# ZhengyiLuo/UHC

Hardware: AMD Instinct MI355X
Metric: env-steps/sec (69-DoF SMPL humanoid, 15 substeps/step) (higher is better)
Workload: dtype f64

## Files before the change

uhc_amd/csrc/uhc_device.h:

```cpp
#pragma once
#include <hip/hip_runtime.h>
#include <stdint.h>

#define UHC_WAVE 64
#define UHC_FAST_MAXEFC 64
#define UHC_FAST_MAXCON 16
#define UHC_FAST_MAXCON_DENSE 24
#define UHC_FAST_MAXTWO 12
#define UHC_GEN_MAXEFC 128
#define UHC_GEN_MAXCON 64
#define UHC_GEN_MAXTWO 20
#define UHC_BIG_MAXEFC 256
#define UHC_BIG_MAXCON 128
#define UHC_BIG_MAXTWO 32
#define UHC_MAXTWO 32
#define UHC_HUGE_MAXEFC 1024
#define UHC_HUGE_MAXCON 192
#define UHC_HUGE_MAXCON_MOST 320
#define UHC_HUGE_MAXTWO 128
#define UHC_DOF_MAXACT 4
#define UHC_CON_STRIDE 24
#define UHC_WHY_CONTACTS (1 << 16)
#define UHC_WHY_ROWS (1 << 17)
#define UHC_WHY_DENSE_SLOTS (1 << 18)
// ... 126 lines not shown
    int last_tier;
    const int* order;
    int tier_want;
    int sticky_mask;
    int* list;
    int* list_count;
    int* list_cursor;
    const int* prod_fin;
    int prod_total;
    int n_wait;
    int* spares;
    int* started;
    int* fin;
    int* q_next;
    int* q_next_count;
    const int* guard_tab;
    int* guard_hits;
    int* cnt4;
    int grid;
    int marks[8];
    int t4_rows;
    int truncate;
    int ball_limits;
    int dbg;
    int nvp;
    int adjdeg;
    DevCtrl c;
    DevState s;
    int n_env;
    int chunk;
    int* ticket;
    int* chunk_done;
    int* chunk_rec;
};
#define UHC_CHUNK_ALL 0x7fff
#define UHC_CHUNK_ABANDON (1 << 30)
#define UHC_CHUNK_TAKEN (1 << 29)
#define UHC_CHUNK_CLOSING (1 << 28)
#define UHC_CHUNK_REC 16
```

uhc_amd/csrc/uhc_mpr.h:

```cpp
#pragma once

#define UHC_CCD_EPS 2.220446049250313e-16
#define UHC_MPR_TOLERANCE 1e-6
#define UHC_MPR_MAXIT 50
#define UHC_MPR_MAXSUP 256

struct V3 { double x, y, z; };
__device__ __forceinline__ V3 v3(double x, double y, double z) { V3 r = {x, y, z}; return r; }
__device__ __forceinline__ V3 operator-(const V3& a, const V3& b) { return v3(a.x - b.x, a.y - b.y, a.z - b.z); }
__device__ __forceinline__ V3 operator+(const V3& a, const V3& b) { return v3(a.x + b.x, a.y + b.y, a.z + b.z); }
__device__ __forceinline__ V3 operator*(const V3& a, double s) { return v3(a.x * s, a.y * s, a.z * s); }
__device__ __forceinline__ V3 neg(const V3& a) { return v3(-a.x, -a.y, -a.z); }
__device__ __forceinline__ double vdot(const V3& a, const V3& b) { return a.x * b.x + a.y * b.y + a.z * b.z; }
__device__ __forceinline__ V3 vcross(const V3& a, const V3& b) { return v3(a.y * b.z - a.z * b.y, a.z * b.x - a.x * b.z, a.x * b.y - a.y * b.x); }
__device__ __forceinline__ V3 vnorm(const V3& a) { const double n = sqrt(vdot(a, a)); return v3(a.x / n, a.y / n, a.z / n); }
__device__ __forceinline__ V3 vsel(bool c, const V3& a, const V3& b) { return v3(c ? a.x : b.x, c ? a.y : b.y, c ? a.z : b.z); }
__device__ __forceinline__ bool ccd_zero(double x) { return fabs(x) < UHC_CCD_EPS; }
__device__ __forceinline__ bool ccd_eq(double a, double b) {
    const double ab = fabs(a - b);
    if (ab < UHC_CCD_EPS) return true;
    a = fabs(a); b = fabs(b);
    return b > a ? ab < UHC_CCD_EPS * b : ab < UHC_CCD_EPS * a;
}

// ... 362 lines not shown
                if (cont) dir = vnorm(vcross(p1.v - p0.v, p2.v - p0.v));
                else { p3 = v4; to_refine = true; }
            }
        } else if (st == MPR_REFINE) {
            dt = vdot(v4.v, dir);
            if (!(ccd_zero(dt) || dt > 0) || portal_reach_tolerance(p1, p2, p3, v4, dir)) st = MPR_DONE;
            else { expand_portal(p0, p1, p2, p3, v4); to_refine = true; }
        } else if (st == MPR_PEN) {
            if (portal_reach_tolerance(p1, p2, p3, v4, dir) || it > UHC_MPR_MAXIT) {
                V3 pd;
                M.depth = sqrt(point_tri_dist2(p1.v, p2.v, p3.v, pd));
                if (ccd_zero(pd.x) && ccd_zero(pd.y) && ccd_zero(pd.z)) pd = dir;
                M.dir = vnorm(pd);
                M.pos = find_pos(p0, p1, p2, p3);
                M.hit = true;
                st = MPR_DONE;
            } else {
                expand_portal(p0, p1, p2, p3, v4);
                it++;
                dir = portal_dir(p1, p2, p3);
            }
        }
        if (to_refine) {
            dir = portal_dir(p1, p2, p3);
            dt = vdot(dir, p1.v);
            if (ccd_zero(dt) || dt > 0) to_pen = true;
            else st = MPR_REFINE;
        }
        if (to_pen) { dir = portal_dir(p1, p2, p3); it = 0; st = MPR_PEN; }
    }
}

#if defined(UHC_NW2)
enum { MCMD_EXIT = 0, MCMD_ROUND = 1, MCMD_ROWS = 2 };
struct MprMB { int* hdr; double* io[6]; double* hm1; double* hm2; int* st4; int* st2; };
template <int TIER>
__device__ __forceinline__ MprMB mpr_mb(const KernelArgs& A, double* S) {
    const DevLds& L = lds_of<TIER>(A);
    MprMB m;
    m.hdr = (int*)(S + L.rowR);
    m.io[0] = S + L.rowR + 4;
    m.io[1] = S + L.rowAref; m.io[2] = S + L.rowAref + UHC_WAVE;
    m.io[3] = S + L.rowB; m.io[4] = S + L.rowB + UHC_WAVE;
    m.io[5] = S + L.rowF; m.hm1 = S + L.rowF + UHC_WAVE;
    m.st4 = (int*)(S + L.rowDa); m.st2 = (int*)(S + L.rowW); m.hm2 = S + L.rowW + UHC_WAVE;
    return m;
}
__device__ __forceinline__ SupArgs mpr_mb_args(const MprMB& MB, const double* xmat, const double* xpos, int p) {
    SupArgs a;
    const int b1 = __builtin_amdgcn_readfirstlane(MB.st4[4 * p]), b2 = __builtin_amdgcn_readfirstlane(MB.st4[4 * p + 1]);
    a.R1 = xmat + 9 * b1; a.P1 = xpos + 3 * b1; a.R2 = xmat + 9 * b2; a.P2 = xpos + 3 * b2;
    a.voff1 = __builtin_amdgcn_readfirstlane(MB.st4[4 * p + 2]); a.vn1 = __builtin_amdgcn_readfirstlane(MB.st4[4 * p + 3]);
    a.voff2 = __builtin_amdgcn_readfirstlane(MB.st2[2 * p]); a.vn2 = __builtin_amdgcn_readfirstlane(MB.st2[2 * p + 1]);
    a.hm1 = MB.hm1[p]; a.hm2 = MB.hm2[p];
    a.d = v3(MB.io[0][p], MB.io[1][p], MB.io[2][p]);
    return a;
}
__device__ __forceinline__ void mpr_mb_put(const MprMB& MB, int p, const V3& a, const V3& b) {
    if (LANE == 0) {
        MB.io[0][p] = a.x - b.x; MB.io[1][p] = a.y - b.y; MB.io[2][p] = a.z - b.z; MB.io[3][p] = a.x + b.x; MB.io[4][p] = a.y + b.y; MB.io[5][p] = a.z + b.z;
    }
}
__device__ __forceinline__ void mpr_serve_round(const double* __restrict__ VB, const double* __restrict__ xmat, const double* __restrict__ xpos, const MprMB& MB, unsigned long long live, int wid, int nw) {
    const int n = __builtin_popcountll(live), h = (n + nw - 1) / nw;
    int take = min(h, n - wid * h);
    for (int k = 0; k < wid * h && live; k++) live &= live - 1;
    while (live && take > 0) {
// ... 88 lines not shown
                }
                if (cont) dir = vnorm(vcross(p1.v - p0.v, p2.v - p0.v));
                else { p3 = v4; to_refine = true; }
            }
        } else if (st == MPR_REFINE) {
            dt = vdot(v4.v, dir);
            if (!(ccd_zero(dt) || dt > 0) || portal_reach_tolerance(p1, p2, p3, v4, dir)) st = MPR_DONE;
            else { expand_portal(p0, p1, p2, p3, v4); to_refine = true; }
        } else if (st == MPR_PEN) {
            if (portal_reach_tolerance(p1, p2, p3, v4, dir) || it > UHC_MPR_MAXIT) {
                V3 pd;
                M.depth = sqrt(point_tri_dist2(p1.v, p2.v, p3.v, pd));
                if (ccd_zero(pd.x) && ccd_zero(pd.y) && ccd_zero(pd.z)) pd = dir;
                M.dir = vnorm(pd);
                M.pos = find_pos(p0, p1, p2, p3);
                M.hit = true;
                st = MPR_DONE;
            } else {
                expand_portal(p0, p1, p2, p3, v4);
                it++;
                dir = portal_dir(p1, p2, p3);
            }
        }
        if (to_refine) {
            dir = portal_dir(p1, p2, p3);
            dt = vdot(dir, p1.v);
            if (ccd_zero(dt) || dt > 0) to_pen = true;
            else st = MPR_REFINE;
        }
        if (to_pen) { dir = portal_dir(p1, p2, p3); it = 0; st = MPR_PEN; }
    }
}
template <int TIER>
__device__ __forceinline__ void mpr_helper(const KernelArgs& A, double* S) {
    const DevLds& L = lds_of<TIER>(A);
    const MprMB MB = mpr_mb<TIER>(A, S);
    const int* mbi = MB.hdr;
    const int wid = __builtin_amdgcn_readfirstlane((int)(threadIdx.x >> 6));
    const LaneConst HLC = lane_const<true>(A.t);
    for (;;) {
        __syncthreads();
        const int cmd = __builtin_amdgcn_readfirstlane(mbi[0]);
        if (cmd == MCMD_EXIT) return;
        if (cmd == MCMD_ROWS) {
            const int nefc = __builtin_amdgcn_readfirstlane(mbi[1]), ntwo = __builtin_amdgcn_readfirstlane(mbi[2]);
            const unsigned long long mbp = ((unsigned long long)(unsigned)__builtin_amdgcn_readfirstlane(mbi[5]) << 32) | (unsigned)__builtin_amdgcn_readfirstlane(mbi[4]);
            __syncthreads();
            if (ntwo > 0) k_dense_groups<TIER>(A, S, HLC, S + L.dense, ntwo, 1, 2);
            __syncthreads();
            if (UHC_WAVE + LANE < nefc) k_row_one<TIER>(A, (const double*)mbp, S, UHC_WAVE + LANE, S + L.Y);
            __syncthreads();
            continue;
        }
        const unsigned long long live = ((unsigned long long)(unsigned)__builtin_amdgcn_readfirstlane(mbi[2]) << 32) | (unsigned)__builtin_amdgcn_readfirstlane(mbi[1]);
        const int vst = __builtin_amdgcn_readfirstlane(mbi[3]);
        if (vst >= 0) mpr_serve_round(S + vst, S + L.xmat, S + L.xpos, MB, live, wid, UHC_NWG);
        else {
            const unsigned long long vb = ((unsigned long long)(unsigned)__builtin_amdgcn_readfirstlane(mbi[5]) << 32) | (unsigned)__builtin_amdgcn_readfirstlane(mbi[4]);
            mpr_serve_round((const double*)vb, S + L.xmat, S + L.xpos, MB, live, wid, UHC_NWG);
        }
        __syncthreads();
    }
}
template <int TIER>
__device__ __forceinline__ void mpr_release_helpers(const KernelArgs& A, double* S) {
    int* mbi = mpr_mb<TIER>(A, S).hdr;
    if (LANE == 0) mbi[0] = MCMD_EXIT;
    __syncthreads();
}
#endif
```

uhc_amd/csrc/uhc_physics_impl.h:

```cpp
#pragma once
#include <type_traits>
#include "../../include/uhc_amd.h"
#include "uhc_device.h"

extern __shared__ __attribute__((aligned(16))) double smem[];

#if defined(UHC_NW4)
#define UHC_NWG 4
#elif defined(UHC_NW2)
#define UHC_NWG 2
#else
#define UHC_NWG 1
#endif
#if UHC_NWG > 1
#define LANE ((int)(threadIdx.x & 63u))
#else
#define LANE ((int)threadIdx.x)
#endif
#define UHC_NPROF 40
#ifdef UHC_STAGE_PROF
#define PROF_DECL long long pt_[UHC_NPROF] = {}; long long pt_last_ = __builtin_readcyclecounter();
#define PROF_ARGS , long long* pt_, long long& pt_last_
#define PROF_PASS , pt_, pt_last_
#define PROF(i) { const long long now_ = __builtin_readcyclecounter(); pt_[i] += now_ - pt_last_; pt_last_ = now_; }
// ... 35 lines not shown
    int lo = __builtin_amdgcn_readlane(__double2loint(v), src);
    int hi = __builtin_amdgcn_readlane(__double2hiint(v), src);
    return __hiloint2double(hi, lo);
}
template <int CTRL>
__device__ __forceinline__ double dpp_f64(double v) {
    const int lo = __builtin_amdgcn_update_dpp(0, __double2loint(v), CTRL, 0xf, 0xf, true);
    const int hi = __builtin_amdgcn_update_dpp(0, __double2hiint(v), CTRL, 0xf, 0xf, true);
    return __hiloint2double(hi, lo);
}
#define DPP_QUAD_1032 0xB1
#define DPP_QUAD_2301 0x4E
#define DPP_ROW_HALF_MIRROR 0x141
#define DPP_ROW_MIRROR 0x140
__device__ __forceinline__ double wave_sum(double v) {
    v += dpp_f64<DPP_QUAD_1032>(v);
    v += dpp_f64<DPP_QUAD_2301>(v);
    v += dpp_f64<DPP_ROW_HALF_MIRROR>(v);
    v += dpp_f64<DPP_ROW_MIRROR>(v);
    return (bcast(v, 0) + bcast(v, 16)) + (bcast(v, 32) + bcast(v, 48));
}
__device__ __forceinline__ double wave_min(double v) {
    v = fmin(v, dpp_f64<DPP_QUAD_1032>(v));
    v = fmin(v, dpp_f64<DPP_QUAD_2301>(v));
    v = fmin(v, dpp_f64<DPP_ROW_HALF_MIRROR>(v));
    v = fmin(v, dpp_f64<DPP_ROW_MIRROR>(v));
    return fmin(fmin(bcast(v, 0), bcast(v, 16)), fmin(bcast(v, 32), bcast(v, 48)));
}
__device__ __forceinline__ int wave_or(int v) { return __builtin_amdgcn_ballot_w64(v != 0) != 0; }
template <int TIER> __device__ __forceinline__ void k_row_one(const KernelArgs& A, const double* mb, double* S, const int r, double* Yb);
struct LaneConst { int d0, d1, n0, n1, m0, m1, pk0, pk1, r0, r1; bool v0, v1; };
template <int TIER> __device__ __forceinline__ void k_dense_groups(const KernelArgs& A, double* S, const LaneConst& LC, double* Db, const int ntwo, const int first, const int stride);
template <bool DENSE> __device__ __forceinline__ LaneConst lane_const(const DevTopo& T);
#include "uhc_mpr.h"

__device__ __forceinline__ void cross3(double* r, const double* a, const double* b) {
    double r0 = a[1] * b[2] - a[2] * b[1], r1 = a[2] * b[0] - a[0] * b[2], r2 = a[0] * b[1] - a[1] * b[0];
    r[0] = r0; r[1] = r1; r[2] = r2;
}
__device__ __forceinline__ double dot3(const double* a, const double* b) { return a[0] * b[0] + a[1] * b[1] + a[2] * b[2]; }
__device__ __forceinline__ void quat_mul(double* r, const double* a, const double* b) {
    double t0 = a[0] * b[0] - a[1] * b[1] - a[2] * b[2] - a[3] * b[3];
    double t1 = a[0] * b[1] + a[1] * b[0] + a[2] * b[3] - a[3] * b[2];
    double t2 = a[0] * b[2] - a[1] * b[3] + a[2] * b[0] + a[3] * b[1];
    double t3 = a[0] * b[3] + a[1] * b[2] - a[2] * b[1] + a[3] * b[0];
    r[0] = t0; r[1] = t1; r[2] = t2; r[3] = t3;
}
__device__ __forceinline__ void quat_normalize(double* q) {
    double n = sqrt(q[0] * q[0] + q[1] * q[1] + q[2] * q[2] + q[3] * q[3]);
    if (n < UHC_MINVAL) { q[0] = 1; q[1] = q[2] = q[3] = 0; return; }
    double inv = 1.0 / n;
    q[0] *= inv; q[1] *= inv; q[2] *= inv; q[3] *= inv;
}
__device__ __forceinline__ void quat_to_mat(double* m, const double* q) {
    double w = q[0], x = q[1], y = q[2], z = q[3];
    m[0] = w * w + x * x - y * y - z * z; m[1] = 2 * (x * y - w * z); m[2] = 2 * (x * z + w * y);
    m[3] = 2 * (x * y + w * z); m[4] = w * w - x * x + y * y - z * z; m[5] = 2 * (y * z - w * x);
    m[6] = 2 * (x * z - w * y); m[7] = 2 * (y * z + w * x); m[8] = w * w - x * x - y * y + z * z;
}
__device__ __forceinline__ void mat_vec(double* r, const double* m, const double* v) {
    double t0 = m[0] * v[0] + m[1] * v[1] + m[2] * v[2];
    double t1 = m[3] * v[0] + m[4] * v[1] + m[5] * v[2];
    double t2 = m[6] * v[0] + m[7] * v[1] + m[8] * v[2];
    r[0] = t0; r[1] = t1; r[2] = t2;
}
__device__ __forceinline__ void axis_angle_quat(double* q, const double* axis, double angle) {
// ... 1524 lines not shown
        unsigned long long Fb = Fm;
        asm volatile("" : "+s"(Fb));
        static_for<0, NC>([&](auto kc) __attribute__((always_inline)) {
            constexpr int k = NC - 1 - decltype(kc)::value;
            if ((Fb >> k) & 1ull) {
                const double xk = bcast(acc * mypinv, k);
                f = ln == k ? xk : f;
                acc = fma(-W[k], xk, acc);
            }
        });
        PROF(27)
        double y = b;
        unsigned long long Fy = Fm;
        asm volatile("" : "+s"(Fy));
        static_for<0, NC>([&](auto sc) __attribute__((always_inline)) {
            constexpr int s = decltype(sc)::value;
            if ((Fy >> s) & 1ull) y = fma(__hiloint2double(agpr_get(Ahi[s]), agpr_get(Alo[s])), bcast(f, s), y);
        });
        PROF(28)
        const bool bad = valid && (inF ? f < 0.0 : y < 0.0);
        const unsigned long long Bm = __builtin_amdgcn_ballot_w64(bad);
        if (Bm == 0ull) { f_out = f; return it; }
        const int nbad = __builtin_popcountll(Bm);
        bool all = true;
        if (nbad < best) { best = nbad; grace = 3; }
        else if (grace > 0) grace--;
        else all = false;
        const int last = 63 - __builtin_clzll(Bm);
        if (bad && (all || LANE == last)) inF = !inF;
    }
    return -1;
}

template <int LT, bool DENSE>
__device__ __forceinline__ int k_pgs_fast(const KernelArgs& A, const double* mb, double* S, int nefc, FastRow& row, const double (&Y)[UHC_YM], const LaneConst& LC,
                                          const int* SL, int nslot PROF_ARGS) {
    const DevTopo& T = A.t;
    const DevLds& L = lds_of<LT>(A);
    const bool valid = LANE < nefc;
    int ntwo = 0;
    if constexpr (DENSE) {
        for (int k = 0; k < nslot; k++) ntwo += (unsigned)SL[k] < (unsigned)nefc;
        ntwo = __builtin_amdgcn_readfirstlane(ntwo);
    }
    if (DENSE && ntwo > 0) {
        unsigned int cdq[UHC_YM];
        const unsigned int* chain = T.chain + (size_t)(row.last >= 0 ? row.last : 0) * UHC_YM;
        static_for<0, UHC_YM>([&](auto qc) __attribute__((always_inline)) { constexpr int q = decltype(qc)::value; cdq[q] = chain[q] & 0xffffu; });
        for (int k = 0; k < nslot; k++) {
            if ((unsigned)__builtin_amdgcn_readfirstlane(SL[k]) >= (unsigned)nefc) continue;
            const double* Dk = S + L.dense + k * A.nvp;
            double acc = 0.0;
            static_for<0, UHC_YM>([&](auto qc) __attribute__((always_inline)) {
                constexpr int q = decltype(qc)::value;
                acc = fma(Y[q], Dk[cdq[q]], acc);
            });
            S[L.dcol + k * UHC_WAVE + LANE] = valid ? acc : 0.0;
        }
        wsync();
        for (int k = 0; k < nslot; k++) {
            const int lk = __builtin_amdgcn_readfirstlane(SL[k]);
            if ((unsigned)lk >= (unsigned)nefc) continue;
            const double* Dk = S + L.dense + k * A.nvp;
            const double dk0 = LC.v0 ? Dk[LANE] : 0.0, dk1 = LC.v1 ? Dk[LANE + UHC_WAVE] : 0.0;
            for (int m = 0; m <= k; m++) {
                const int lm = __builtin_amdgcn_readfirstlane(SL[m]);
                if ((unsigned)lm >= (unsigned)nefc) continue;
                const double* Dm = S + L.dense + m * A.nvp;
                const double v = wave_sum(dk0 * (LC.v0 ? Dm[LANE] : 0.0) + dk1 * (LC.v1 ? Dm[LANE + UHC_WAVE] : 0.0));
                if (LANE == 0) { S[L.dcol + k * UHC_WAVE + lm] = v; S[L.dcol + m * UHC_WAVE + lk] = v; }
            }
        }
        wsync();
    }
    unsigned int ncp[UHC_WAVE / 4];
    {
        int nraw[UHC_WAVE];
        static_for<0, UHC_WAVE>([&](auto sc) __attribute__((always_inline)) {
            constexpr int s = decltype(sc)::value;
            nraw[s] = 0;
            if (s < nefc) {
                const int ls = __builtin_amdgcn_readlane(row.last, s);
                nraw[s] = (valid && row.last >= 0 && ls >= 0) ? (int)A.t.dof_ncommon[row.last * T.nv + ls] : 0;
            }
        });
        static_for<0, UHC_WAVE / 4>([&](auto jc) __attribute__((always_inline)) {
            constexpr int j = decltype(jc)::value;
            ncp[j] = (unsigned)nraw[4 * j] | ((unsigned)nraw[4 * j + 1] << 8) | ((unsigned)nraw[4 * j + 2] << 16) | ((unsigned)nraw[4 * j + 3] << 24);
        });
    }
    double Ym[UHC_YM];
    int Alo[UHC_WAVE], Ahi[UHC_WAVE];
    double diag = 1.0;
    int prev = -1;
    static_for<0, UHC_YM>([&](auto qc) __attribute__((always_inline)) { Ym[decltype(qc)::value] = 0.0; });
    auto build_A = [&](auto dense_c) __attribute__((always_inline)) {
    constexpr bool DCOL = decltype(dense_c)::value;
    static_for<0, UHC_WAVE>([&](auto sc) __attribute__((always_inline)) {
        constexpr int s = decltype(sc)::value;
        double acc = 0.0;
        if (s < nefc) {
            const int ls = __builtin_amdgcn_readlane(row.last, s);
            const int lens = __builtin_amdgcn_readlane(row.len, s);
            const int two_s = DCOL ? __builtin_amdgcn_readlane(row.two, s) : -1;
            if (DCOL && two_s >= 0) acc = S[L.dcol + two_s * UHC_WAVE + LANE];
            else {
            const double* Ys = S + L.Y + __builtin_amdgcn_readlane(row.yoff, s);
            if (ls != prev) {
                prev = ls;
                const int nc = (ncp[s / 4] >> (8 * (s % 4))) & 0xff;
                static_for<0, UHC_YM>([&](auto qc) __attribute__((always_inline)) {
                    constexpr int q = decltype(qc)::value;
                    Ym[q] = q < nc ? Y[q] : 0.0;
                });
            }
            static_for<0, UHC_YM / 8>([&](auto cc) __attribute__((always_inline)) {
                constexpr int c = decltype(cc)::value;
                if (8 * c < lens) {
                    double y8[8];
                    static_for<0, 8>([&](auto qc) __attribute__((always_inline)) { constexpr int j = decltype(qc)::value; y8[j] = Ys[8 * c + j]; });
                    static_for<0, 8>([&](auto qc) __attribute__((always_inline)) {
                        constexpr int j = decltype(qc)::value;
                        acc = fma(Ym[8 * c + j], y8[j], acc);
// ... 92 lines not shown
    const double f = row.f;
    PROF(11)
    for (int i = LANE; i < T.nv; i += UHC_WAVE) S[L.z + i] = 0.0;
    wsync();
    if (valid && row.last >= 0) {
        const unsigned int* chain = T.chain + (size_t)row.last * UHC_YM;
        const double* Yr = S + L.Y + row.yoff;
        static_for<0, UHC_YM>([&](auto qc) __attribute__((always_inline)) {
            constexpr int q = decltype(qc)::value;
            if (q < row.len) __hip_atomic_fetch_add(S + L.z + (chain[q] & 0xffffu), f * Yr[q], __ATOMIC_RELAXED, __HIP_MEMORY_SCOPE_WORKGROUP);
        });
    }
    wsync();
    if (DENSE && ntwo > 0) {
        for (int k = 0; k < nslot; k++) {
            const int ln = __builtin_amdgcn_readfirstlane(SL[k]);
            if ((unsigned)ln >= (unsigned)nefc) continue;
            const double fk = bcast(f, ln);
            const double* Dk = S + L.dense + k * A.nvp;
            if (LC.v0) S[L.z + LANE] += fk * Dk[LANE];
            if (LC.v1) S[L.z + LANE + UHC_WAVE] += fk * Dk[LANE + UHC_WAVE];
        }
        wsync();
    }
    return iters;
}

#define UHC_WS_MAXIT 16
#define UHC_WS_BLOCK_MAXIT 80
#define UHC_WS_LOST_MAXIT 6
#define UHC_WS_WINDOWED 0x10000
#define UHC_WS_FILL 64
#define UHC_LOST_SWEEPS 32
template <int TIER, bool DENSE>
__device__ __forceinline__ int k_as_general(const KernelArgs& A, const double* mb, double* S, int nefc, const LaneConst& LC, bool lost PROF_ARGS) {
    constexpr int NRL = TIER == 3 ? 4 : 2;
    const DevTopo& T = A.t;
    const DevLds& L = lds_of<TIER>(A);
    const RowMisc* RM = (const RowMisc*)(S + L.rowMisc);
    const int* RY = (const int*)(S + L.rowY);
    const int YS = T.maxdepth + 1;
    int* NI = (int*)(S + L.ncon_nefc);
    const int nslot = (DENSE && cap_of<TIER>(A).ndense > 0) ? NI[2] : 0;
    int* SLg = NI + 4 + UHC_MAXTWO;
    int* list = (int*)(S + L.rowAref);
    double* z = S + L.z;
    const unsigned long long below = (1ull << LANE) - 1ull;
    int rr[NRL];
    bool vv[NRL];
    bool fric = false;
#pragma unroll
    for (int h = 0; h < NRL; h++) {
        rr[h] = LANE + h * UHC_WAVE;
        vv[h] = rr[h] < nefc;
        fric = fric || (vv[h] && RTYPE(RM[rr[h]].type) == ROW_FRICTION);
    }
    if (wave_or(fric)) return -1;
    double pr[NRL];
#pragma unroll
    for (int h = 0; h < NRL; h++) pr[h] = vv[h] ? S[L.rowAref + rr[h]] : 1e300;
    wsync();
#pragma unroll
    for (int h = 0; h < NRL; h++) if (vv[h]) S[L.rowW + rr[h]] = S[L.rowF + rr[h]];
    for (int i = LANE; i < T.nv; i += UHC_WAVE) z[i] = 0.0;
    wsync();
    int* label = list + UHC_WAVE;
// ... 211 lines not shown
                        const double* Dk = S + L.dense + k * A.nvp;
                        if (LC.v0) zfix[LANE] += fk * Dk[LANE];
                        if (LC.v1) zfix[LANE + UHC_WAVE] += fk * Dk[LANE + UHC_WAVE];
                    }
                    wsync();
                }
                if (valid) {
                    double yb = 0.0;
                    if (two) {
                        const double* D = S + L.dense + row.two * A.nvp;
                        for (int i = 0; i < T.nv; i++) yb = fma(D[i], zfix[i], yb);
                    } else {
                        const short* anc = T.dof_anc + rm.last * YS;
                        const double* Yr = S + L.Y + row.yoff;
                        for (int k = 0; k < row.len; k++) yb = fma(Yr[k], zfix[anc[k]], yb);
                    }
                    row.b += yb;
                }
            }
            PROF(30)
            const int it = k_pgs_fast<TIER, DENSE>(A, mb, S, nC, row, Y, LC, SLg, nslot PROF_PASS);
            if (it < 0) return -4;
            iters += it > 0 ? it : 1;
            if (block) {
                for (int i = LANE; i < T.nv; i += UHC_WAVE) z[i] += zfix[i];
                wsync();
            }
#pragma unroll
            for (int h = 0; h < NRL; h++) if (in[h] && !fx[h]) S[L.rowF + rr[h]] = 0.0;
            wsync();
            if (valid) S[L.rowF + r] = row.f;
            wsync();
            bool viol[NRL], keep[NRL], anyv = false;
#pragma unroll
            for (int h = 0; h < NRL; h++) {
                viol[h] = keep[h] = false;
                if (!in[h]) continue;
                if (c[h]) { keep[h] = S[L.rowF + rr[h]] > 0.0; continue; }
                const RowMisc q = RM[rr[h]];
                double y = S[L.rowB + rr[h]];
                if (q.type & ROW_TWO) {
                    const double* D = S + L.dense + (q.type >> 8) * A.nvp;
                    for (int i = 0; i < T.nv; i++) y = fma(D[i], z[i], y);
                } else {
                    const int len = T.dof_depth[q.last] + 1;
                    const short* anc = T.dof_anc + q.last * YS;
                    const double* Yr = S + L.Y + RY[rr[h]];
                    for (int k = 0; k < len; k++) y = fma(Yr[k], z[anc[k]], y);
                }
                if (fx[h]) y = fma(S[L.rowR + rr[h]], S[L.rowF + rr[h]], y);
                viol[h] = fx[h] ? fabs(y) > tol : y < -tol;
                anyv = anyv || viol[h];
            }
            PROF(31)
            if (!wave_or(anyv)) {
                for (int i = LANE; i < T.nv; i += UHC_WAVE) ztot[i] += z[i];
                wsync();
                done = true;
            } else {
#pragma unroll
                for (int h = 0; h < NRL; h++) { c[h] = keep[h] || viol[h] || fx[h]; p[h] = keep[h] || fx[h]; }
                wsync();
            }
        }
        if (split) { todo |= G; nomerge = true; continue; }
        if (!done) return -3;
    }
    for (int i = LANE; i < T.nv; i += UHC_WAVE) z[i] = ztot[i];
    wsync();
    return iters | (windowed ? UHC_WS_WINDOWED : 0);
}

template <int TIER>
__device__ __forceinline__ int k_primal(const KernelArgs& A, const double* mb, double* S, int nefc, const LaneConst& LC, const double* Yb, const double* Db, int* nact PROF_ARGS);
#ifdef UHC_WITH_TIER4
#include "uhc_primal.h"
#endif

struct FwdOut { int ncon, nefc, iters, overflow, nact, ytot; };
#define UHC_POISON_BITS 0x7ff8dead7fffbeefll
template <int TIER>
__device__ __forceinline__ void guard_arm(const KernelArgs& A, double* S) {
#ifdef UHC_GUARD_LDS
    if (!A.guard_tab) return;
    const int* g = A.guard_tab + 64 * (TIER - 1);
    wsync();
// ... 684 lines not shown
```

uhc_amd/csrc/uhc_plan.cpp:

```cpp
#include "uhc_plan.h"

#include <algorithm>
#include <cstdarg>
#include <cstdio>
#include <cstdlib>
#include <cstring>

static int refuse(std::string* err, const char* fmt, ...) {
    char buf[1024];
    va_list ap;
    va_start(ap, fmt);
    vsnprintf(buf, sizeof buf, fmt, ap);
    va_end(ap);
    *err = buf;
    return 1;
}

BatchKnobs read_knobs() {
    BatchKnobs k;
    auto is = [](const char* name, char c) { const char* e = getenv(name); return e && e[0] == c; };
    auto at_least = [](const char* name, int lo, int* v) { if (const char* e = getenv(name)) *v = std::max(lo, atoi(e)); };
    k.guard = is("UHC_GUARD_LDS", '2') ? 2 : is("UHC_GUARD_LDS", '1') ? 1 : 0;
    if (const char* dbg = getenv("UHC_DEBUG")) k.dbg = atoi(dbg);
    if (k.guard) k.dbg |= 2;
#ifndef UHC_EXPERIMENTS
    k.dbg &= ~0x1f00;
#endif
    if (const char* m = getenv("UHC_TIER_MARKS")) sscanf(m, "%d,%d,%d,%d,%d,%d,%d,%d", k.marks, k.marks + 1, k.marks + 2, k.marks + 3, k.marks + 4, k.marks + 5, k.marks + 6, k.marks + 7);
    if (const char* fd = getenv("UHC_FAST_DENSE")) k.fast_dense_got = sscanf(fd, "%d,%d,%d", &k.fast_dense_kib, &k.fast_dense_rows, &k.fast_dense_con);
    k.fast_dcol_own = is("UHC_FAST_DCOL_OWN", '1');
    if (const char* pad = getenv("UHC_LDS_PAD_FAST")) { k.lds_pad_fast = true; k.lds_pad_fast_kib = atoi(pad); }
    k.force_general = is("UHC_FORCE_GENERAL", '1');
    k.tiers = is("UHC_TIERS", '2') ? 2 : is("UHC_TIERS", '3') ? 3 : 0;
    at_least("UHC_Q2_DIV", 1, &k.q2_div); at_least("UHC_Q2_WAIT", 1, &k.q2_wait_min); at_least("UHC_Q2_MAX", 16, &k.q2_max);
    at_least("UHC_Q3_MAX", 2, &k.q3_max); at_least("UHC_Q4_MAX", 0, &k.q4_max); at_least("UHC_T4_ROWS", 0, &k.t4_rows);
    if (const char* fc = getenv("UHC_FAST_CHUNK")) {
        char* end = nullptr;
        const long v = strtol(fc, &end, 10);
        if (end == fc || *end != 0 || v < 0) k.fast_chunk_bad = true;
        else k.fast_chunk = (v == 0 || v > 0x7fff) ? 0x7fff : (int)v;
    }
    return k;
}

static bool same_topology(const UhcModelDesc& a, const UhcModelDesc& b) {
    if (a.nq != b.nq || a.nv != b.nv || a.nu != b.nu || a.nbody != b.nbody || a.njnt != b.njnt || a.ngeom != b.ngeom ||
        a.nmeshvert != b.nmeshvert || a.nexclude != b.nexclude)
        return false;
    auto eq = [](const int32_t* x, const int32_t* y, size_t n) { return !memcmp(x, y, n * 4); };
    return eq(a.body_parentid, b.body_parentid, a.nbody) && eq(a.jnt_type, b.jnt_type, a.njnt) &&
           eq(a.jnt_bodyid, b.jnt_bodyid, a.njnt) && eq(a.dof_parentid, b.dof_parentid, a.nv) &&
           eq(a.geom_type, b.geom_type, a.ngeom) && eq(a.geom_bodyid, b.geom_bodyid, a.ngeom) &&
           eq(a.geom_vertadr, b.geom_vertadr, a.ngeom) && eq(a.geom_vertnum, b.geom_vertnum, a.ngeom) &&
           eq(a.geom_contype, b.geom_contype, a.ngeom) && eq(a.geom_conaffinity, b.geom_conaffinity, a.ngeom) &&
           eq(a.jnt_limited, b.jnt_limited, a.njnt) && eq(a.geom_condim, b.geom_condim, a.ngeom);
}

static void build_blob(const UhcModelDesc& d, DevNumOff& o, std::vector<double>& blob, int adjdeg) {
    blob.clear();
    auto put = [&](const double* p, size_t n) { int off = (int)blob.size(); blob.insert(blob.end(), p, p + n); return off; };
    o.body_pos = put(d.body_pos, 3 * d.nbody); o.body_quat = put(d.body_quat, 4 * d.nbody);
    o.body_ipos = put(d.body_ipos, 3 * d.nbody); o.body_iquat = put(d.body_iquat, 4 * d.nbody);
    o.body_mass = put(d.body_mass, d.nbody); o.body_inertia = put(d.body_inertia, 3 * d.nbody);
    o.body_invweight0 = put(d.body_invweight0, 2 * d.nbody);
    o.jnt_pos = put(d.jnt_pos, 3 * d.njnt); o.jnt_axis = put(d.jnt_axis, 3 * d.njnt); o.jnt_range = put(d.jnt_range, 2 * d.njnt);
    o.jnt_stiffness = put(d.jnt_stiffness, d.njnt); o.jnt_margin = put(d.jnt_margin, d.njnt);
    o.qpos0 = put(d.qpos0, d.nq); o.qpos_spring = put(d.qpos_spring, d.nq);
    o.dof_armature = put(d.dof_armature, d.nv); o.dof_damping = put(d.dof_damping, d.nv);
// ... 427 lines not shown
            const int i = nv - 1 - s2;
            P.sol_back[(size_t)s2 * 64 + l] = entry(i, l) | (entry(i, l + 64) << 16);
            P.sol_fwd[(size_t)s2 * 64 + l] = entry(l, s2) | (entry(l + 64, s2) << 16);
        }
    P.chain.assign((size_t)nv * 32, adr(0) << 16);
    for (int i = 0; i < nv; i++)
        for (int q = 0; q <= dof_depth[i]; q++) {
            const int a = P.dof_anc[(size_t)i * YS + q];
            P.chain[(size_t)i * 32 + q] = (unsigned)a | (adr(d.dof_madr[a]) << 16);
        }
    return 0;
}

static int actuator_table(const UhcModelDesc& d, BatchPlan& P, std::string* err) {
    P.dof_act.assign((size_t)d.nv * UHC_DOF_MAXACT, -1);
    for (int a = 0; a < d.nu; a++) {
        const int j = d.dof_jntid[d.actuator_dofid[a]], nd = d.jnt_type[j] == UHC_JNT_BALL ? 3 : d.jnt_type[j] == UHC_JNT_FREE ? 6 : 1;
        if (nd == 6) return refuse(err, "uhc_batch_create: motors on free joints are not supported");
        for (int k = 0; k < nd; k++) {
            int q = 0;
            while (q < UHC_DOF_MAXACT && P.dof_act[(size_t)(d.jnt_dofadr[j] + k) * UHC_DOF_MAXACT + q] >= 0) q++;
            if (q == UHC_DOF_MAXACT) return refuse(err, "uhc_batch_create: more than %d motors on one joint", UHC_DOF_MAXACT);
            P.dof_act[(size_t)(d.jnt_dofadr[j] + k) * UHC_DOF_MAXACT + q] = a;
        }
    }
    return 0;
}

#define PLAN_TRY(x) do { if (x) return 1; } while (0)
int plan_batch(const UhcModel* const* models, int n_models, const int32_t* env_model, int n_env, const UhcCtrlDesc* ctrl, const BatchKnobs& knobs,
               BatchPlan* out, std::string* err) {
    BatchPlan& P = *out;
    P = BatchPlan();
    if (knobs.fast_chunk_bad) return refuse(err, "uhc_batch_create: UHC_FAST_CHUNK must be a non-negative integer (substeps per chunk of the fast tier's control step)");
    PLAN_TRY(validate(models, n_models, env_model, n_env, ctrl, &P.n_trailing_free, err));
    const UhcModelDesc& d = models[0]->d;
    KernelArgs& A = P.A;
    memset(&A, 0, sizeof A);
    DevTopo& T = A.t;
    const int nv = d.nv;
    T.nq = d.nq; T.nv = nv; T.nu = d.nu; T.nbody = d.nbody; T.njnt = d.njnt; T.ngeom = d.ngeom; T.nmeshvert = d.nmeshvert;
    T.nM = d.dof_madr[nv];
    T.iterations = d.iterations; T.plane_mesh_maxcon = d.plane_mesh_maxcon; T.solver = d.solver;
    T.timestep = d.timestep; T.tolerance = d.tolerance;
    for (int k = 0; k < 3; k++) T.gravity[k] = d.gravity[k];
    T.has_damping = 0;
    for (int k = 0; k < n_models; k++)
        for (int i = 0; i < nv; i++) T.has_damping |= models[k]->d.dof_damping[i] > 0;
    for (int j = 0; j < d.njnt; j++) A.ball_limits |= d.jnt_type[j] == UHC_JNT_BALL && d.jnt_limited[j] != 0;
    A.n_env = n_env;
    tree_tables(d, P);
    PLAN_TRY(validate_trees(d, P, err));
    PLAN_TRY(collision_pairs(d, P, err));
    PLAN_TRY(model_blobs(models, n_models, P, err));
    PLAN_TRY(controller(d, ctrl, P, err));
    if (T.nM > 64 * 24) return refuse(err, "uhc_batch_create: nM %d > 1536 (the register tile that carries M between substeps)", T.nM);
    A.nvp = (nv + 1) & ~1;
    A.dbg = knobs.dbg;
    A.t4_rows = knobs.t4_rows;
    for (int k = 0; k < 8; k++) A.marks[k] = knobs.marks[k];
    Carver cv[4];
    for (Carver& c : cv) c.guard_on = knobs.guard != 0;
    fast_layout(cv[0], d, n_env, knobs, P);
    PLAN_TRY(upper_tiers(cv, d, knobs, P, err));
    if (knobs.guard) PLAN_TRY(guard_table(cv, knobs, P, err));
    PLAN_TRY(schedules(d, P, err));
    PLAN_TRY(actuator_table(d, P, err));
    return 0;
}

FastChunks plan_fast_chunks(int n_substeps, int chunk, int n_env) {
    FastChunks f;
    f.chunk = (chunk <= 0 || chunk >= n_substeps) ? 0 : chunk;
    f.n_chunks = f.chunk ? (n_substeps + f.chunk - 1) / f.chunk : 1;
    f.grid = f.n_chunks * n_env;
    f.prod_total = f.grid;
    return f;
}
void fast_chunk_range(const FastChunks& f, int n_substeps, int c, int* lo, int* hi) {
    *lo = f.chunk ? c * f.chunk : 0;
    *hi = f.chunk ? std::min(*lo + f.chunk, n_substeps) : n_substeps;
}
#define UHC_FAST_CHUNK_DEFAULT 5
int default_fast_chunk(int knob, int n_substeps, int n_env, int n_cu, size_t lds_bytes_fast) {
    if (knob > 0) return knob >= n_substeps ? 0 : knob;
    const int per_cu = std::max(1, std::min(4, (int)(160 * 1024 / std::max<size_t>(lds_bytes_fast, 1))));
    return (n_env > per_cu * n_cu && UHC_FAST_CHUNK_DEFAULT < n_substeps) ? UHC_FAST_CHUNK_DEFAULT : 0;
}

StickySizes plan_sticky_step(const StickyInputs& in) {
    StickySizes s;
// ... 22 lines not shown
```

uhc_amd/csrc/uhc_plan.h:

```cpp
#pragma once
#include <string>
#include <vector>

#include "uhc_host.h"

struct BatchKnobs {
    int dbg = 0;
    int marks[8] = {64, 16, -1, 56, 14, 10, 8, 7};
    int fast_dense_got = 0, fast_dense_kib = 0, fast_dense_rows = 0, fast_dense_con = 0;
    bool fast_dcol_own = false;
    bool lds_pad_fast = false;
    int lds_pad_fast_kib = 0;
    bool force_general = false;
    int tiers = 0;
    int guard = 0;
    int q2_div = 1, q2_wait_min = 16, q2_max = 256, q3_max = 32, q4_max = 16;
    int t4_rows = 0;
    int fast_chunk = 0;
    bool fast_chunk_bad = false;
};
BatchKnobs read_knobs();

struct BatchPlan {
    KernelArgs A;
    size_t lds_bytes = 0, lds_bytes_fast = 0, lds_bytes_big = 0;
    bool use_fast = true;
    int n_trailing_free = 0;
    std::vector<int> body_depth, body_rootid, body_nsub, body_lastdof, dof_depth, dof_ndesc, dof_rootid;
    std::vector<short> dof_anc, m_row, m_col;
    std::vector<unsigned short> m_ij;
    std::vector<unsigned char> ncommon;
    std::vector<int> pg1, pg2, cg1, cg2;
    std::vector<double> model_blob;
    std::vector<unsigned int> fac_prog, sol_back, sol_fwd, chain;
    std::vector<int> dof_act;
    std::vector<int> vf_body;
    std::vector<int> guard_tab;
};
int plan_batch(const UhcModel* const* models, int n_models, const int32_t* env_model, int n_env, const UhcCtrlDesc* ctrl, const BatchKnobs& knobs,
               BatchPlan* out, std::string* err);

struct StickyInputs {
    int est2, est3, est4;
    int est2_then;
    int handed2;
    int n_env, n_cu;
    size_t lds_bytes_fast;
    bool large_first;
    int last_tier;
    bool queues_off;
// ... 21 lines not shown
```

Before: 101,700.

## Share general-tier dense pair products and working-set row checks with helper wave

```diff
diff --git a/uhc_amd/csrc/uhc_device.h b/uhc_amd/csrc/uhc_device.h
--- a/uhc_amd/csrc/uhc_device.h
+++ b/uhc_amd/csrc/uhc_device.h
@@ -182,6 +182,7 @@
     int* ticket;
     int* chunk_done;
     int* chunk_rec;
+    int gen_split;
 };
 #define UHC_CHUNK_ALL 0x7fff
 #define UHC_CHUNK_ABANDON (1 << 30)
diff --git a/uhc_amd/csrc/uhc_mpr.h b/uhc_amd/csrc/uhc_mpr.h
--- a/uhc_amd/csrc/uhc_mpr.h
+++ b/uhc_amd/csrc/uhc_mpr.h
@@ -418,7 +418,8 @@
 }
 
 #if defined(UHC_NW2)
-enum { MCMD_EXIT = 0, MCMD_ROUND = 1, MCMD_ROWS = 2 };
+enum { MCMD_EXIT = 0, MCMD_ROUND = 1, MCMD_ROWS = 2, MCMD_PAIRS = 3, MCMD_YROWS = 4 };
+static_assert(UHC_GEN_MAXEFC <= 2 * UHC_WAVE && UHC_GEN_MAXEFC >= 128, "the two-wave consumer's helper takes the rows 64 .. 127 (MCMD_ROWS, MCMD_YROWS)");
 struct MprMB { int* hdr; double* io[6]; double* hm1; double* hm2; int* st4; int* st2; };
 template <int TIER>
 __device__ __forceinline__ MprMB mpr_mb(const KernelArgs& A, double* S) {
@@ -573,6 +574,21 @@
     }
 }
 template <int TIER>
+__device__ __forceinline__ void gs_post(const KernelArgs& A, double* S, int cmd, int a1, int a2, int a3, int a4, double d) {
+    const DevLds& L = lds_of<TIER>(A);
+    int* mbi = (int*)(S + L.rowR);
+    static_assert(UHC_WAVE + 1 + 4 <= UHC_GEN_MAXEFC, "gs_post parks rowR[0 .. 3] in rowAref[UHC_WAVE + 1 .. UHC_WAVE + 4]");
+    double* keep = S + L.rowAref + UHC_WAVE + 1;
+    if (LANE < 4) keep[LANE] = S[L.rowR + LANE];
+    wsync();
+    if (LANE == 0) { mbi[0] = cmd; mbi[1] = a1; mbi[2] = a2; mbi[3] = a3; mbi[4] = a4; S[L.rowR + 3] = d; }
+    __syncthreads();
+    __syncthreads();
+    if (LANE < 4) S[L.rowR + LANE] = keep[LANE];
+    wsync();
+}
+__device__ __forceinline__ void gs_join() { __syncthreads(); }
+template <int TIER>
 __device__ __forceinline__ void mpr_helper(const KernelArgs& A, double* S) {
     const DevLds& L = lds_of<TIER>(A);
     const MprMB MB = mpr_mb<TIER>(A, S);
@@ -593,6 +609,22 @@
             __syncthreads();
             continue;
         }
+        if (cmd == MCMD_PAIRS || cmd == MCMD_YROWS) {
+            const int a1 = __builtin_amdgcn_readfirstlane(mbi[1]), a2 = __builtin_amdgcn_readfirstlane(mbi[2]), a3 = __builtin_amdgcn_readfirstlane(mbi[3]), a4 = __builtin_amdgcn_readfirstlane(mbi[4]);
+            const double tol = __hiloint2double(__builtin_amdgcn_readfirstlane(mbi[7]), __builtin_amdgcn_readfirstlane(mbi[6]));
+            __syncthreads();
+            if (cmd == MCMD_PAIRS) k_dense_pairs<TIER>(A, S, HLC, (const int*)(S + L.ncon_nefc) + 4 + UHC_MAXTWO, a2, a1, 1, 2);
+            else {
+                const unsigned long long todo = ((unsigned long long)(unsigned)a2 << 32) | (unsigned)a1, held = ((unsigned long long)(unsigned)a4 << 32) | (unsigned)a3;
+                bool v = false;
+                if ((todo >> LANE) & 1ull) v = ws_row_violated<TIER>(A, S, UHC_WAVE + LANE, ((held >> LANE) & 1ull) != 0, tol);
+                const unsigned long long vm = __builtin_amdgcn_ballot_w64(v);
+                int* res = (int*)(S + L.rowAref) + 2 * UHC_WAVE;
+                if (LANE == 0) { res[0] = (int)(vm & 0xffffffffull); res[1] = (int)(vm >> 32); }
+            }
+            __syncthreads();
+            continue;
+        }
         const unsigned long long live = ((unsigned long long)(unsigned)__builtin_amdgcn_readfirstlane(mbi[2]) << 32) | (unsigned)__builtin_amdgcn_readfirstlane(mbi[1]);
         const int vst = __builtin_amdgcn_readfirstlane(mbi[3]);
         if (vst >= 0) mpr_serve_round(S + vst, S + L.xmat, S + L.xpos, MB, live, wid, UHC_NWG);
diff --git a/uhc_amd/csrc/uhc_physics_impl.h b/uhc_amd/csrc/uhc_physics_impl.h
--- a/uhc_amd/csrc/uhc_physics_impl.h
+++ b/uhc_amd/csrc/uhc_physics_impl.h
@@ -91,6 +91,8 @@
 struct LaneConst { int d0, d1, n0, n1, m0, m1, pk0, pk1, r0, r1; bool v0, v1; };
 template <int TIER> __device__ __forceinline__ void k_dense_groups(const KernelArgs& A, double* S, const LaneConst& LC, double* Db, const int ntwo, const int first, const int stride);
 template <bool DENSE> __device__ __forceinline__ LaneConst lane_const(const DevTopo& T);
+template <int LT> __device__ __forceinline__ void k_dense_pairs(const KernelArgs& A, double* S, const LaneConst& LC, const int* SL, int nslot, int nefc, int first, int stride);
+template <int TIER> __device__ __forceinline__ bool ws_row_violated(const KernelArgs& A, const double* S, int r, bool fx, double tol);
 #include "uhc_mpr.h"
 
 __device__ __forceinline__ void cross3(double* r, const double* a, const double* b) {
@@ -1681,6 +1683,27 @@
     return -1;
 }
 
+#define UHC_SPLIT_MINTWO 4
+template <int LT>
+__device__ __forceinline__ void k_dense_pairs(const KernelArgs& A, double* S, const LaneConst& LC, const int* SL, int nslot, int nefc, int first, int stride) {
+    const DevLds& L = lds_of<LT>(A);
+    int idx = 0;
+    for (int k = 0; k < nslot; k++) {
+        const int lk = __builtin_amdgcn_readfirstlane(SL[k]);
+        if ((unsigned)lk >= (unsigned)nefc) continue;
+        const double* Dk = S + L.dense + k * A.nvp;
+        const double dk0 = LC.v0 ? Dk[LANE] : 0.0, dk1 = LC.v1 ? Dk[LANE + UHC_WAVE] : 0.0;
+        for (int m = 0; m <= k; m++) {
+            const int lm = __builtin_amdgcn_readfirstlane(SL[m]);
+            if ((unsigned)lm >= (unsigned)nefc) continue;
+            if (stride > 1 && (idx++ % stride) != first) continue;
+            const double* Dm = S + L.dense + m * A.nvp;
+            const double v = wave_sum(dk0 * (LC.v0 ? Dm[LANE] : 0.0) + dk1 * (LC.v1 ? Dm[LANE + UHC_WAVE] : 0.0));
+            if (LANE == 0) { S[L.dcol + k * UHC_WAVE + lm] = v; S[L.dcol + m * UHC_WAVE + lk] = v; }
+        }
+    }
+}
+
 template <int LT, bool DENSE>
 __device__ __forceinline__ int k_pgs_fast(const KernelArgs& A, const double* mb, double* S, int nefc, FastRow& row, const double (&Y)[UHC_YM], const LaneConst& LC,
                                           const int* SL, int nslot PROF_ARGS) {
@@ -1692,6 +1715,11 @@
         for (int k = 0; k < nslot; k++) ntwo += (unsigned)SL[k] < (unsigned)nefc;
         ntwo = __builtin_amdgcn_readfirstlane(ntwo);
     }
+    bool shared = false;
+#if defined(UHC_NW2)
+    if constexpr (LT == 2 && DENSE) shared = A.gen_split != 0 && ntwo >= UHC_SPLIT_MINTWO;
+    if (shared) gs_post<LT>(A, S, MCMD_PAIRS, nefc, nslot, 0, 0, 0.0);
+#endif
     if (DENSE && ntwo > 0) {
         unsigned int cdq[UHC_YM];
         const unsigned int* chain = T.chain + (size_t)(row.last >= 0 ? row.last : 0) * UHC_YM;
@@ -1704,23 +1732,13 @@
                 constexpr int q = decltype(qc)::value;
                 acc = fma(Y[q], Dk[cdq[q]], acc);
             });
-            S[L.dcol + k * UHC_WAVE + LANE] = valid ? acc : 0.0;
+            if (!(shared && valid && row.two >= 0)) S[L.dcol + k * UHC_WAVE + LANE] = valid ? acc : 0.0;
         }
         wsync();
-        for (int k = 0; k < nslot; k++) {
-            const int lk = __builtin_amdgcn_readfirstlane(SL[k]);
-            if ((unsigned)lk >= (unsigned)nefc) continue;
-            const double* Dk = S + L.dense + k * A.nvp;
-            const double dk0 = LC.v0 ? Dk[LANE] : 0.0, dk1 = LC.v1 ? Dk[LANE + UHC_WAVE] : 0.0;
-            for (int m = 0; m <= k; m++) {
-                const int lm = __builtin_amdgcn_readfirstlane(SL[m]);
-                if ((unsigned)lm >= (unsigned)nefc) continue;
-                const double* Dm = S + L.dense + m * A.nvp;
-                const double v = wave_sum(dk0 * (LC.v0 ? Dm[LANE] : 0.0) + dk1 * (LC.v1 ? Dm[LANE + UHC_WAVE] : 0.0));
-                if (LANE == 0) { S[L.dcol + k * UHC_WAVE + lm] = v; S[L.dcol + m * UHC_WAVE + lk] = v; }
-            }
-        }
-        wsync();
+        PROF(36)
+        k_dense_pairs<LT>(A, S, LC, SL, nslot, nefc, 0, shared ? 2 : 1);
+        if (!shared) wsync();
+        PROF(37)
     }
     unsigned int ncp[UHC_WAVE / 4];
     {
@@ -1738,6 +1756,10 @@
             ncp[j] = (unsigned)nraw[4 * j] | ((unsigned)nraw[4 * j + 1] << 8) | ((unsigned)nraw[4 * j + 2] << 16) | ((unsigned)nraw[4 * j + 3] << 24);
         });
     }
+#if defined(UHC_NW2)
+    if (shared) gs_join();
+#endif
+    PROF(38)
     double Ym[UHC_YM];
     int Alo[UHC_WAVE], Ahi[UHC_WAVE];
     double diag = 1.0;
@@ -1896,6 +1918,25 @@
 #define UHC_WS_WINDOWED 0x10000
 #define UHC_WS_FILL 64
 #define UHC_LOST_SWEEPS 32
+template <int TIER>
+__device__ __forceinline__ bool ws_row_violated(const KernelArgs& A, const double* S, int r, bool fx, double tol) {
+    const DevTopo& T = A.t;
+    const DevLds& L = lds_of<TIER>(A);
+    const double* z = S + L.z;
+    const RowMisc q = ((const RowMisc*)(S + L.rowMisc))[r];
+    double y = S[L.rowB + r];
+    if (q.type & ROW_TWO) {
+        const double* D = S + L.dense + (q.type >> 8) * A.nvp;
+        for (int i = 0; i < T.nv; i++) y = fma(D[i], z[i], y);
+    } else {
+        const int len = T.dof_depth[q.last] + 1;
+        const short* anc = T.dof_anc + q.last * (T.maxdepth + 1);
+        const double* Yr = S + L.Y + ((const int*)(S + L.rowY))[r];
+        for (int k = 0; k < len; k++) y = fma(Yr[k], z[anc[k]], y);
+    }
+    if (fx) y = fma(S[L.rowR + r], S[L.rowF + r], y);
+    return fx ? fabs(y) > tol : y < -tol;
+}
 template <int TIER, bool DENSE>
 __device__ __forceinline__ int k_as_general(const KernelArgs& A, const double* mb, double* S, int nefc, const LaneConst& LC, bool lost PROF_ARGS) {
     constexpr int NRL = TIER == 3 ? 4 : 2;
@@ -2173,26 +2214,35 @@
             if (valid) S[L.rowF + r] = row.f;
             wsync();
             bool viol[NRL], keep[NRL], anyv = false;
+            bool yshared = false;
+#if defined(UHC_NW2)
+            if constexpr (TIER == 2) {
+                const unsigned long long ym = __builtin_amdgcn_ballot_w64(in[1] && !c[1]);
+                yshared = A.gen_split != 0 && ym != 0ull;
+                if (yshared) {
+                    const unsigned long long hm = __builtin_amdgcn_ballot_w64(fx[1]);
+                    gs_post<TIER>(A, S, MCMD_YROWS, (int)(ym & 0xffffffffull), (int)(ym >> 32), (int)(hm & 0xffffffffull), (int)(hm >> 32), tol);
+                }
+            }
+#endif
 #pragma unroll
             for (int h = 0; h < NRL; h++) {
                 viol[h] = keep[h] = false;
                 if (!in[h]) continue;
                 if (c[h]) { keep[h] = S[L.rowF + rr[h]] > 0.0; continue; }
-                const RowMisc q = RM[rr[h]];
-                double y = S[L.rowB + rr[h]];
-                if (q.type & ROW_TWO) {
-                    const double* D = S + L.dense + (q.type >> 8) * A.nvp;
-                    for (int i = 0; i < T.nv; i++) y = fma(D[i], z[i], y);
-                } else {
-                    const int len = T.dof_depth[q.last] + 1;
-                    const short* anc = T.dof_anc + q.last * YS;
-                    const double* Yr = S + L.Y + RY[rr[h]];
-                    for (int k = 0; k < len; k++) y = fma(Yr[k], z[anc[k]], y);
-                }
-                if (fx[h]) y = fma(S[L.rowR + rr[h]], S[L.rowF + rr[h]], y);
-                viol[h] = fx[h] ? fabs(y) > tol : y < -tol;
+                if (yshared && h == 1) continue;
+                viol[h] = ws_row_violated<TIER>(A, S, rr[h], fx[h], tol);
                 anyv = anyv || viol[h];
             }
+#if defined(UHC_NW2)
+            if constexpr (TIER == 2) if (yshared) {
+                gs_join();
+                const int* res = (const int*)(S + L.rowAref) + 2 * UHC_WAVE;
+                const unsigned long long vm = ((unsigned long long)(unsigned)res[1] << 32) | (unsigned)res[0];
+                viol[1] = in[1] && !c[1] && ((vm >> LANE) & 1ull) != 0;
+                anyv = anyv || viol[1];
+            }
+#endif
             PROF(31)
             if (!wave_or(anyv)) {
                 for (int i = LANE; i < T.nv; i += UHC_WAVE) ztot[i] += z[i];
diff --git a/uhc_amd/csrc/uhc_plan.cpp b/uhc_amd/csrc/uhc_plan.cpp
--- a/uhc_amd/csrc/uhc_plan.cpp
+++ b/uhc_amd/csrc/uhc_plan.cpp
@@ -34,6 +34,10 @@
     k.tiers = is("UHC_TIERS", '2') ? 2 : is("UHC_TIERS", '3') ? 3 : 0;
     at_least("UHC_Q2_DIV", 1, &k.q2_div); at_least("UHC_Q2_WAIT", 1, &k.q2_wait_min); at_least("UHC_Q2_MAX", 16, &k.q2_max);
     at_least("UHC_Q3_MAX", 2, &k.q3_max); at_least("UHC_Q4_MAX", 0, &k.q4_max); at_least("UHC_T4_ROWS", 0, &k.t4_rows);
+    if (const char* gs = getenv("UHC_GEN_SPLIT")) {
+        if (gs[0] == '0' && gs[1] == 0) k.gen_split = false;
+        else if (!(gs[0] == '1' && gs[1] == 0)) k.gen_split_bad = true;
+    }
     if (const char* fc = getenv("UHC_FAST_CHUNK")) {
         char* end = nullptr;
         const long v = strtol(fc, &end, 10);
@@ -527,6 +531,7 @@
                BatchPlan* out, std::string* err) {
     BatchPlan& P = *out;
     P = BatchPlan();
+    if (knobs.gen_split_bad) return refuse(err, "uhc_batch_create: UHC_GEN_SPLIT must be 0 or 1 (the helper wave's share of the general tier's working-set solve)");
     if (knobs.fast_chunk_bad) return refuse(err, "uhc_batch_create: UHC_FAST_CHUNK must be a non-negative integer (substeps per chunk of the fast tier's control step)");
     PLAN_TRY(validate(models, n_models, env_model, n_env, ctrl, &P.n_trailing_free, err));
     const UhcModelDesc& d = models[0]->d;
@@ -552,6 +557,7 @@
     if (T.nM > 64 * 24) return refuse(err, "uhc_batch_create: nM %d > 1536 (the register tile that carries M between substeps)", T.nM);
     A.nvp = (nv + 1) & ~1;
     A.dbg = knobs.dbg;
+    A.gen_split = knobs.gen_split ? 1 : 0;
     A.t4_rows = knobs.t4_rows;
     for (int k = 0; k < 8; k++) A.marks[k] = knobs.marks[k];
     Carver cv[4];
diff --git a/uhc_amd/csrc/uhc_plan.h b/uhc_amd/csrc/uhc_plan.h
--- a/uhc_amd/csrc/uhc_plan.h
+++ b/uhc_amd/csrc/uhc_plan.h
@@ -16,6 +16,8 @@
     int guard = 0;
     int q2_div = 1, q2_wait_min = 16, q2_max = 256, q3_max = 32, q4_max = 16;
     int t4_rows = 0;
+    bool gen_split = true;
+    bool gen_split_bad = false;
     int fast_chunk = 0;
     bool fast_chunk_bad = false;
 };
```

After: 104,000 (median of 6 runs). 2.2% higher.
